# gizatechxyz/LuminAIR

Hardware: AMD Instinct MI355X
Metric: proofs/sec, 2^20-row Add trace (higher is better)
Workload: dtype u32 (M31/QM31 field arithmetic)

## Files before the change

### luminair_amd/csrc/fft_fixed.h

```cpp
#pragma once
#include "kernels.h"

namespace lmn {

bool launch_fft_fixed_pass(bool inverse, uint32_t* data, uint64_t col_stride, const uint32_t* src, uint64_t src_stride, int lo,
                           int rbits, int cb, int log_n, const TwPtrs& tw, uint32_t scale_log, int ncols, int cpb,
                           uint32_t h_off, int xcd_swizzle, bool zero_extended_top, lmn_stream_t s);
bool launch_interp_extend_fixed(uint32_t* coeffs, uint64_t coeff_stride, uint32_t* lde, uint64_t lde_stride, int log_n,
                                const TwPtrs& itw, const TwPtrs& tw_ext, int ncols, lmn_stream_t s);
bool launch_fft_rows_fixed(uint32_t* coeffs, uint64_t col_stride, const uint32_t* rows, uint64_t n_rows, int ncols, int log_n,
                           const PadRow& pad, uint32_t* bad_flag, uint32_t bad_value, const TwPtrs& itw, lmn_stream_t s);

}
```

### luminair_amd/csrc/fft_fixed.hip

```cpp
#include "fft_fixed.h"

#include <algorithm>

#include "issue_phases.h"
#include "launch_util.h"

namespace lmn {

LMN_HD constexpr uint32_t fx_pad(uint32_t e) { return e + (e >> 5); }

#if !defined(LMN_EMU) && !defined(LMN_BATCH)
#define LMN_BOUNDS(n) __launch_bounds__(n)
#else
#define LMN_BOUNDS(n)
#endif

struct GTile {
#if defined(__HIP_DEVICE_COMPILE__) && !defined(LMN_EMU)
  __amdgpu_buffer_rsrc_t r;
#else
  uint32_t* p;
#endif
};
LMN_D GTile gtile(const uint32_t* p) {
// ... 254 lines not shown
}

struct TwD {
  const uint32_t* l[MAX_LOG];
};
static TwD doubled(const TwPtrs& tw) {
  TwD t{};
  for (int i = 0; i < MAX_LOG; ++i) t.l[i] = tw.d[i];
  return t;
}

template <bool INV, int RBITS, int CB, bool LO0, bool ZX = false>
LMN_KERNEL LMN_BOUNDS((FxShape<RBITS, CB, LO0>::NT))
k_fft_fx(uint32_t* data, uint64_t col_stride, const uint32_t* src, uint64_t src_stride, int lo_arg, TwD tw, uint32_t scale_log,
         int ncols, int cpb, uint32_t h_off, int xcd_swizzle) {
  using S = FxShape<RBITS, CB, LO0>;
  LMN_DYN_SMEM(uint32_t, sm);
  const int lo = LO0 ? 0 : lo_arg;
  uint32_t tile = blockIdx.x;
  if (xcd_swizzle && (gridDim.x & 7u) == 0u) tile = (blockIdx.x & 7u) * (gridDim.x >> 3) + (blockIdx.x >> 3);
  const uint32_t q = tile & ((1u << (lo - CB)) - 1u);
  const uint32_t Hl = tile >> (lo - CB);
  const uint64_t base = ((uint64_t)Hl << (lo + RBITS)) + ((uint64_t)q << CB);
  const uint32_t H = Hl + h_off;
  for (int cc = 0; cc < cpb; ++cc) {
    const int c = (int)blockIdx.y * cpb + cc;
    if (c >= ncols) break;
    uint32_t* col = data + (uint64_t)c * col_stride + base;
    const uint32_t* scol = src + (uint64_t)c * src_stride + base;
    fx_steps<S, INV, 0, true, true, false, ZX>(sm, sm, col, scol, lo, H, tw.l, scale_log, nullptr, threadIdx.x);
  }
}

template <int RBITS>
LMN_KERNEL LMN_BOUNDS((FxShape<RBITS, 4, false>::NT))
k_fft_interp_extend_fx(uint32_t* coeffs, uint64_t coeff_stride, uint32_t* lde, uint64_t lde_stride, TwD itw, TwD tw,
                       uint32_t scale_log) {
  using S = FxShape<RBITS, 4, false>;
  constexpr int LO = 12;
  LMN_DYN_SMEM(uint32_t, sm);
  uint32_t* A = sm;
  uint32_t* B = sm + S::LDS_WORDS;
  uint32_t tile = blockIdx.x;
  if ((gridDim.x & 7u) == 0u) tile = (blockIdx.x & 7u) * (gridDim.x >> 3) + (blockIdx.x >> 3);
  const uint64_t base = (uint64_t)tile << 4;
  const uint64_t n_words = 1ull << (LO + RBITS);
  uint32_t* ccol = coeffs + (uint64_t)blockIdx.y * coeff_stride + base;
  uint32_t* lcol = lde + (uint64_t)blockIdx.y * lde_stride + base;
  fx_steps<S, true, 0, true, true, true>(B, B, ccol, ccol, LO, 0u, itw.l, scale_log, A, threadIdx.x);
  for (uint32_t h = 0; h < 2; ++h)
    fx_steps<S, false, 0, false, true, false>(A, B, lcol + h * n_words, nullptr, LO, h, tw.l, 0u, nullptr, threadIdx.x);
}

template <int COLS>
LMN_KERNEL LMN_BOUNDS((COLS / 2) * 256)
k_fft_rows_fx(uint32_t* coeffs, uint64_t col_stride, const uint32_t* __restrict__ rows, uint64_t n_rows, int ncols, PadRow pad,
              uint32_t* __restrict__ bad_flag, uint32_t bad_value, TwD itw, uint32_t n_groups) {
  using S = FxShape<12, 0, true>;
  constexpr uint32_t NT = (uint32_t)S::NT, TILE = 1u << 12, GROUPS = COLS / 2;
  static_assert(NT == 256, "one lane group per tile");
  LMN_DYN_SMEM(uint32_t, sm);
  uint32_t tile = blockIdx.x / n_groups, ygrp = blockIdx.x % n_groups;
  if ((gridDim.x & 7u) == 0u && ((gridDim.x / n_groups) & 7u) == 0u) {
    const uint32_t x = blockIdx.x & 7u, sq = blockIdx.x >> 3;
    tile = (sq / n_groups) * 8u + x;
    ygrp = sq % n_groups;
  }
  const int c0 = (int)ygrp * COLS;
  const int ncb = ncols - c0 < COLS ? ncols - c0 : COLS;
  const uint64_t row0 = (uint64_t)tile << 12;
  {
    constexpr int BATCH = 8;
    constexpr uint32_t CELLS = TILE * COLS, STEP = GROUPS * NT;
    for (uint32_t k0 = threadIdx.x; k0 < CELLS; k0 += BATCH * STEP) {
      uint32_t v[BATCH];
#pragma unroll
      for (int j = 0; j < BATCH; ++j) {
        const uint32_t k = k0 + (uint32_t)j * STEP;
        const uint32_t r = k / COLS, c = k % COLS;
        const uint64_t gr = row0 + r;
        v[j] = 0u;
        if ((int)c < ncb) v[j] = gr < n_rows ? rows[gr * (uint64_t)ncols + (uint32_t)c0 + c] : pad.v[(uint32_t)c0 + c];
      }
#pragma unroll
// ... 82 lines not shown
    switch (rbits) {
      case 5: LMN_FX_CASE(5, 5, false);
      case 6: LMN_FX_CASE(6, 5, false);
      case 7: LMN_FX_CASE(7, 5, false);
      default: return false;
    }
  }
  if (cb == 4 && lo >= 4) {
    switch (rbits) {
      case 6: LMN_FX_CASE(6, 4, false);
      case 7: LMN_FX_CASE(7, 4, false);
      case 8: LMN_FX_CASE(8, 4, false);
      case 9: LMN_FX_CASE(9, 4, false);
      case 10: LMN_FX_CASE(10, 4, false);
      default: return false;
    }
  }
  return false;
#undef LMN_FX_CASE
}

bool launch_fft_fixed_pass(bool inverse, uint32_t* data, uint64_t col_stride, const uint32_t* src, uint64_t src_stride, int lo,
                           int rbits, int cb, int log_n, const TwPtrs& tw, uint32_t scale_log, int ncols, int cpb,
                           uint32_t h_off, int xcd_swizzle, bool zero_extended_top, lmn_stream_t s) {
  static const bool off = env_set("LMN_NO_FFT_FIXED");
  if (off || !tw.d[0]) return false;
  if (zero_extended_top && (inverse || lo + rbits != log_n)) return false;
  return inverse ? dispatch_fx<true>(data, col_stride, src, src_stride, lo, rbits, cb, log_n, tw, scale_log, ncols, cpb, h_off,
                                     xcd_swizzle, false, s)
                 : dispatch_fx<false>(data, col_stride, src, src_stride, lo, rbits, cb, log_n, tw, scale_log, ncols, cpb, h_off,
                                      xcd_swizzle, zero_extended_top, s);
}

template <int RBITS>
static void launch_ie(uint32_t* coeffs, uint64_t coeff_stride, uint32_t* lde, uint64_t lde_stride, const TwPtrs& itw,
                      const TwPtrs& tw_ext, uint32_t scale_log, int ncols, lmn_stream_t s) {
  using S = FxShape<RBITS, 4, false>;
  const size_t smem = (size_t)8 * S::LDS_WORDS;
#if !defined(LMN_EMU) && !defined(LMN_BATCH)
  if (smem > 64 * 1024) allow_big_lds((const void*)k_fft_interp_extend_fx<RBITS>, 160 * 1024);
#endif
  LMN_LAUNCH((k_fft_interp_extend_fx<RBITS>), dim3(1u << (12 - 4), (unsigned)ncols), dim3(S::NT), smem, s, coeffs, coeff_stride,
             lde, lde_stride, doubled(itw), doubled(tw_ext), scale_log);
}

bool launch_interp_extend_fixed(uint32_t* coeffs, uint64_t coeff_stride, uint32_t* lde, uint64_t lde_stride, int log_n,
                                const TwPtrs& itw, const TwPtrs& tw_ext, int ncols, lmn_stream_t s) {
  static const bool off = env_set("LMN_NO_FFT_FIXED");
  if (off || !itw.d[0] || !tw_ext.d[0]) return false;
  const uint32_t scale_log = (uint32_t)((31 - (log_n % 31)) % 31);
  switch (log_n - 12) {
    case 6: launch_ie<6>(coeffs, coeff_stride, lde, lde_stride, itw, tw_ext, scale_log, ncols, s); return true;
    case 7: launch_ie<7>(coeffs, coeff_stride, lde, lde_stride, itw, tw_ext, scale_log, ncols, s); return true;
    case 8: launch_ie<8>(coeffs, coeff_stride, lde, lde_stride, itw, tw_ext, scale_log, ncols, s); return true;
    case 9: launch_ie<9>(coeffs, coeff_stride, lde, lde_stride, itw, tw_ext, scale_log, ncols, s); return true;
    default: return false;
  }
}

}
```

### luminair_amd/csrc/kernels.h

```cpp
#pragma once
#include "blake2s.h"
#include "field.h"

namespace lmn {

constexpr int MAX_LOG = 30;

struct TwPtrs {
  const uint32_t* l[MAX_LOG];
  const uint32_t* d[MAX_LOG];
};

struct PadRow {
  uint32_t v[32];
};
void launch_transpose_pad(const uint32_t* rows, uint64_t n_rows, int ncols, int log_size, uint32_t* cols,
                          const PadRow& pad, uint32_t* bad_flag , lmn_stream_t s);
void launch_transpose_pad_rows(const uint32_t* rows, uint64_t n_rows, int ncols, int log_size, uint32_t* cols,
                               uint64_t out_stride, uint64_t blk_row0, uint64_t blk_rows, const PadRow& pad, uint32_t* bad_flag,
                               lmn_stream_t s,
                               uint32_t bad_value = 1u );
constexpr int CHUNK_ROWS = 256;
constexpr int CHUNK_MAX_COLS = 30;
void launch_rows_chunk(const uint32_t* chunk, uint64_t r0, uint64_t n, int ncols, uint32_t* cols, uint64_t stride,
                       const PadRow& pad, uint32_t* bad_word, lmn_stream_t s);
constexpr int PREPARE_MAX_LUT_COLS = 6;
struct PrepareCols {
  const uint32_t* lut[PREPARE_MAX_LUT_COLS];
  uint32_t n[PREPARE_MAX_LUT_COLS];
  int n_luts;
  uint32_t* range_check;
  uint32_t range_n;
};
void launch_settings_prepare(const PrepareCols& cols, uint32_t* flag, lmn_stream_t s);

int launch_ifft(uint32_t* dst, uint64_t dst_stride, const uint32_t* src, uint64_t src_stride, int ncols, int log_n,
                const TwPtrs& itw, lmn_stream_t s);
int launch_fft(uint32_t* dst, uint64_t dst_stride, const uint32_t* src, uint64_t src_stride, int log_src, int ncols,
               int log_n, const TwPtrs& tw, lmn_stream_t s);
bool fft_interp_extend_supported(int log_n);
int launch_interp_extend(uint32_t* coeffs, uint64_t coeff_stride, const uint32_t* evals, uint64_t evals_stride, uint32_t* lde,
                         uint64_t lde_stride, int ncols, int log_n, const TwPtrs& itw, const TwPtrs& tw_ext, lmn_stream_t s);
struct PadRow;
bool launch_interp_extend_rows(uint32_t* coeffs, uint64_t coeff_stride, const uint32_t* rows, uint64_t n_rows, const PadRow& pad,
                               uint32_t* bad_flag, uint32_t bad_value, uint32_t* lde, uint64_t lde_stride, int ncols, int log_n,
                               const TwPtrs& itw, const TwPtrs& tw_ext, lmn_stream_t s);
int launch_fft_block(uint32_t* dst, uint64_t dst_stride, const uint32_t* src, uint64_t src_stride, int log_src, int ncols,
                     int log_n, int log_blocks, uint32_t block, const TwPtrs& tw, lmn_stream_t s);
struct PackSel {
  uint32_t blk[8][2];
};
void launch_pack_blocks(const uint32_t* src, uint64_t src_stride, uint32_t* dst, uint32_t block_rows, int ncols, int nsel,
                        int world, const PackSel& sel, lmn_stream_t s);
void launch_unpack_blocks(const uint32_t* packed, uint32_t* cols, uint64_t col_stride, uint32_t block_rows, int ncols, int world,
                          lmn_stream_t s);
void launch_fft_simple(uint32_t* data, uint64_t col_stride, int ncols, int log_n, const TwPtrs& tw, bool inverse,
                       lmn_stream_t s);
void launch_extend(const uint32_t* src, uint64_t src_stride, int log_src, uint32_t* dst, uint64_t dst_stride,
                   int log_dst, int ncols, lmn_stream_t s);

void launch_bit_reverse(uint32_t* data, uint64_t col_stride, int ncols, int log_n, lmn_stream_t s);
int decompose_num_blocks(int log_n);
void launch_decompose(const uint32_t* f, int log_n, uint32_t* g, QM31* lambda_out, QM31* scratch, lmn_stream_t s);
void launch_batch_inverse_m31(const uint32_t* src, uint32_t* dst, uint64_t col_stride, int ncols, int log_n,
                              unsigned long long* n_zero, lmn_stream_t s);
void launch_batch_inverse_qm31(const uint32_t* src, uint32_t* dst, int log_n, unsigned long long* n_zero, lmn_stream_t s);

void launch_merkle_layer(const uint32_t* prev, const uint32_t* const* cols, int ncols, uint32_t size, uint32_t* out,
                         lmn_stream_t s);

struct DevChannel {
  uint32_t digest[8];
  uint32_t n_sent;
  uint32_t variant;
};
// ... 263 lines not shown
  uint32_t n;
};
int logup_num_blocks(uint32_t n);
void launch_logup_fracs(const LogupArgs& a, lmn_stream_t s);
void launch_logup_reduce(const uint32_t* partials, int nblocks, uint32_t n_inv, QM31* claimed_out, lmn_stream_t s);
void launch_logup_scan(const QM31* last_tmp, QM31* claimed_shift, int log_size, uint32_t* out_cols ,
                       QM31* blocksums, lmn_stream_t s, bool derive_claim = false, uint32_t n_inv = 0);
int logup_scan_num_blocks(int log_size);

struct CompositionArgs {
  int kind;
  int log_size;
  int eval_log;
  uint32_t row0, n_rows;
  uint64_t stride;
  const uint32_t* main;
  const uint32_t* inter;
  const uint32_t* prev_last;
  uint32_t* out;
  int accumulate;
  QM31 z, alpha;
  QM31 z2, alpha2;
  const DevElems* d_elems;
  int es2;
  const uint32_t* pre;
  const uint32_t* pre2;
  const QM31* claimed_shift;
  QM31 coeff[16];
  const QM31* d_coeff;
  uint32_t zinv[2];
};
void launch_composition(const CompositionArgs& a, lmn_stream_t s);
void launch_secure_add(uint32_t* out, const uint32_t* in, uint64_t n_words, lmn_stream_t s);

struct EvalJob {
  const uint32_t* coeffs;
  int log_n;
  int point;
  int owner = -1;
};
constexpr int EVAL_LB = 10;
void launch_eval_at_point(const EvalJob* jobs, int njobs, const QM31* lo_tab, const QM31* hi_tab, uint32_t hi_stride,
                          int max_log, QM31* partial_out , int max_chunks, lmn_stream_t s,
                          uint32_t shard_rank = 0, uint32_t shard_world = 1);
int eval_num_chunks(int log_n);
void launch_eval_tables(const QM31* maps, int maps_stride, int npoints, QM31* lo_tab, QM31* hi_tab, uint32_t hi_n,
                        int hi_bits, lmn_stream_t s);
void launch_eval_reduce(const EvalJob* jobs, int njobs, const QM31* partial, int max_chunks, QM31* out,
                        lmn_stream_t s);

constexpr int QUOT_MAX_BATCH = 4;
constexpr int QUOT_MAX_ENTRIES = 512;
struct QuotEntry {
  const uint32_t* col;
  QM31 c;
};
struct QuotDev {
  QM31 A[QUOT_MAX_BATCH], B[QUOT_MAX_BATCH], batch_coeff[QUOT_MAX_BATCH];
  CM31 prx[QUOT_MAX_BATCH], pry[QUOT_MAX_BATCH], pix[QUOT_MAX_BATCH], piy[QUOT_MAX_BATCH];
};
struct QuotientArgs {
  int log_size;
  uint32_t row0;
  int log_rows;
  uint64_t out_stride;
  int nbatch;
// ... 44 lines not shown
```

### luminair_amd/csrc/kernels_fft.hip

```cpp
#include "kernels_common.h"

namespace lmn {

constexpr int FFT_MAX_STAGES = 4;
struct FftStagePlan {
  int lo, hi, cb;
  int nst;
  int first[FFT_MAX_STAGES];
  int R[FFT_MAX_STAGES];
  int xcd_swizzle;
};

LMN_HD uint32_t fft_lds_pad(uint32_t e) { return e + (e >> 5); }

template <int N>
LMN_D void m_mul_phased(const uint32_t (&x)[N], const uint32_t (&w)[N], uint32_t (&out)[N]) {
  uint64_t pr[N];
  uint32_t hi[N], s[N], s2[N];
  LMN_PHASE_PORT0();
#pragma unroll
  for (int k = 0; k < N; ++k) pr[k] = (uint64_t)x[k] * (uint64_t)w[k];
#pragma unroll
  for (int k = 0; k < N; ++k) hi[k] = (uint32_t)(pr[k] >> 31);
  LMN_PHASE_ANY();
// ... 179 lines not shown
    case 2: fft_stage<2, INV>(sm_in, sm_out, col, scol, src_len, base, lo, hi, cb, first_layer, H, from_global, to_global, tw, scale, keep); break;
    case 3: fft_stage<3, INV>(sm_in, sm_out, col, scol, src_len, base, lo, hi, cb, first_layer, H, from_global, to_global, tw, scale, keep); break;
    default: fft_stage<4, INV>(sm_in, sm_out, col, scol, src_len, base, lo, hi, cb, first_layer, H, from_global, to_global, tw, scale, keep); break;
  }
}

template <bool INV>
LMN_KERNEL k_fft_staged(uint32_t* data, uint64_t col_stride, const uint32_t* src, uint64_t src_stride,
                        uint64_t src_len, FftStagePlan pl, TwPtrs tw, uint32_t scale, int ncols, int cpb,
                        uint32_t h_off) {
  LMN_DYN_SMEM(uint32_t, sm);
  uint32_t tile = blockIdx.x;
  if (pl.xcd_swizzle && (gridDim.x & 7u) == 0u) tile = (blockIdx.x & 7u) * (gridDim.x >> 3) + (blockIdx.x >> 3);
  const uint32_t q = tile & ((1u << (pl.lo - pl.cb)) - 1u);
  const uint32_t Hl = tile >> (pl.lo - pl.cb);
  const uint64_t base = ((uint64_t)Hl << pl.hi) + ((uint64_t)q << pl.cb);
  const uint32_t H = Hl + h_off;
  for (int cc = 0; cc < cpb; ++cc) {
    const int c = blockIdx.y * cpb + cc;
    if (c >= ncols) break;
    uint32_t* col = data + (uint64_t)c * col_stride;
    const uint32_t* scol = src + (uint64_t)c * src_stride;
    for (int k = 0; k < pl.nst; ++k) {
      const int s = INV ? k : pl.nst - 1 - k;
      const bool fg = k == 0, tg = k == pl.nst - 1;
      fft_stage_dispatch<INV>(pl.R[s], sm, sm, col, scol, src_len, base, pl.lo, pl.hi, pl.cb, pl.first[s], H, fg, tg, tw, scale);
      __syncthreads();
    }
  }
}

LMN_KERNEL k_fft_interp_extend(uint32_t* coeffs, uint64_t coeff_stride, const uint32_t* src, uint64_t src_stride,
                               uint32_t* lde, uint64_t lde_stride, FftStagePlan pl, TwPtrs itw, TwPtrs tw, uint32_t scale,
                               int ncols, int cpb) {
  LMN_DYN_SMEM(uint32_t, sm);
  const uint32_t tile_elems = 1u << (pl.hi - pl.lo + pl.cb);
  uint32_t* A = sm;
  uint32_t* B = sm + fft_lds_pad(tile_elems) + 1u;
  uint32_t tile = blockIdx.x;
  if (pl.xcd_swizzle && (gridDim.x & 7u) == 0u) tile = (blockIdx.x & 7u) * (gridDim.x >> 3) + (blockIdx.x >> 3);
  const uint64_t base = (uint64_t)tile << pl.cb;
  const uint64_t n_words = 1ull << pl.hi;
  for (int cc = 0; cc < cpb; ++cc) {
    const int c = blockIdx.y * cpb + cc;
    if (c >= ncols) break;
    uint32_t* ccol = coeffs + (uint64_t)c * coeff_stride;
    const uint32_t* scol = src + (uint64_t)c * src_stride;
    uint32_t* lcol = lde + (uint64_t)c * lde_stride;
    for (int k = 0; k < pl.nst; ++k) {
      const bool fg = k == 0, tg = k == pl.nst - 1;
      fft_stage_dispatch<true>(pl.R[k], B, B, ccol, scol, n_words, base, pl.lo, pl.hi, pl.cb, pl.first[k], 0u, fg, tg, itw, scale,
                               tg ? A : nullptr);
      __syncthreads();
    }
    for (uint32_t h = 0; h < 2; ++h) {
      for (int k = 0; k < pl.nst; ++k) {
        const int s = pl.nst - 1 - k;
        const bool tg = k == pl.nst - 1;
        fft_stage_dispatch<false>(pl.R[s], k == 0 ? A : B, B, lcol + h * n_words, lcol, 0, base, pl.lo, pl.hi, pl.cb, pl.first[s], h,
                                  false, tg, tw, 1u);
        __syncthreads();
      }
    }
  }
}

struct FftPass {
  int lo, hi, cb;
};
constexpr int FFT_LOW_BITS = 12;
constexpr int FFT_HIGH_BITS = 10;
constexpr int FFT_HIGH_CB = 4;

static int plan_passes(int log_n, FftPass* out) {
  int n = 0;
  int lo = 0;
  int hi = log_n < FFT_LOW_BITS ? log_n : FFT_LOW_BITS;
  out[n++] = {0, hi, 0};
  lo = hi;
  while (lo < log_n) {
    int rem = log_n - lo;
    int npass = (rem + FFT_HIGH_BITS - 1) / FFT_HIGH_BITS;
    int take = (rem + npass - 1) / npass;
    out[n++] = {lo, lo + take, (take == 5 || (npass > 1 && take <= 7)) ? 5 : FFT_HIGH_CB};
    lo += take;
  }
  return n;
}
// ... 38 lines not shown
    const uint32_t scale_log = scale == 1u ? 0u : (uint32_t)__builtin_ctz(scale);
    if (launch_fft_fixed_pass(INV, data, col_stride, psrc, pstride, p.lo, rbits, p.cb, log_n, tw, scale_log, ncols, cpb,
                              block_index << (log_n - p.hi), pl.xcd_swizzle, !full, s))
      return;
  }
  unsigned gy = (unsigned)((ncols + cpb - 1) / cpb);
  const int threads = (int)std::min<uint32_t>(TPB, std::max<uint32_t>(64u, tile_elems >> 4));
  LMN_LAUNCH(k_fft_staged<INV>, dim3(tiles, gy), dim3(threads), smem, s, data, col_stride, psrc, pstride, plen, pl, tw,
             scale, ncols, cpb, block_index << (log_n - p.hi));
}

template <bool INV>
static int run_fft(uint32_t* data, uint64_t col_stride, const uint32_t* src, uint64_t src_stride, int log_src,
                    int ncols, int log_n, const TwPtrs& tw, lmn_stream_t s, uint32_t block_index = 0) {
  if (log_n < 1) throw LmnError(-100, "fft: log_n < 1");
  FftPass passes[8];
  int np = plan_passes(log_n, passes);
  for (int k = 0; k < np; ++k) {
    const FftPass& p = INV ? passes[k] : passes[np - 1 - k];
    bool last = INV && k == np - 1;
    uint32_t scale = last ? inv_pow2(log_n) : 1u;
    const uint32_t* psrc = k == 0 ? src : data;
    uint64_t pstride = k == 0 ? src_stride : col_stride;
    uint64_t plen = k == 0 ? (1ull << log_src) : (1ull << log_n);
    launch_staged_pass<INV>(data, col_stride, psrc, pstride, plen, p, log_n, tw, scale, ncols, s, block_index);
  }
  return np;
}

bool fft_interp_extend_supported(int log_n) {
  static const bool off = env_set("LMN_NO_FFT_FUSION");
  return !off && log_n > FFT_LOW_BITS && log_n - FFT_LOW_BITS <= FFT_HIGH_BITS - 1;
}
static void interp_extend_tail(uint32_t* coeffs, uint64_t coeff_stride, uint32_t* lde, uint64_t lde_stride, int ncols, int log_n,
                               const TwPtrs& itw, const TwPtrs& tw_ext, lmn_stream_t s) {
  const FftPass low{0, FFT_LOW_BITS, 0};
  FftStagePlan pl{};
  pl.lo = FFT_LOW_BITS;
  pl.hi = log_n;
  pl.cb = FFT_HIGH_CB;
  split_stages(pl);
  pl.xcd_swizzle = 1;
  const uint32_t tile_elems = 1u << (log_n - FFT_LOW_BITS + FFT_HIGH_CB);
  const size_t smem = (size_t)8 * (tile_elems + (tile_elems >> 5) + 1);
  const unsigned tiles = 1u << (FFT_LOW_BITS - FFT_HIGH_CB);
  int cpb = 1;
  const int threads = (int)std::min<uint32_t>(TPB, std::max<uint32_t>(64u, tile_elems >> 4));
#if !defined(LMN_EMU) && !defined(LMN_BATCH)
  if (smem > 64 * 1024) allow_big_lds((const void*)k_fft_interp_extend, 160 * 1024);
#endif
  if (!launch_interp_extend_fixed(coeffs, coeff_stride, lde, lde_stride, log_n, itw, tw_ext, ncols, s))
    LMN_LAUNCH(k_fft_interp_extend, dim3(tiles, (unsigned)((ncols + cpb - 1) / cpb)), dim3(threads), smem, s, coeffs,
               coeff_stride, coeffs, coeff_stride, lde, lde_stride, pl, itw, tw_ext, inv_pow2(log_n), ncols, cpb);
  launch_staged_pass<false>(lde, lde_stride, lde, lde_stride, 2ull << log_n, low, log_n + 1, tw_ext, 1u, ncols, s);
}

int launch_interp_extend(uint32_t* coeffs, uint64_t coeff_stride, const uint32_t* evals, uint64_t evals_stride, uint32_t* lde,
                         uint64_t lde_stride, int ncols, int log_n, const TwPtrs& itw, const TwPtrs& tw_ext, lmn_stream_t s) {
  if (!fft_interp_extend_supported(log_n)) throw LmnError(-100, "interp_extend: unsupported size");
  const FftPass low{0, FFT_LOW_BITS, 0};
  launch_staged_pass<true>(coeffs, coeff_stride, evals, evals_stride, 1ull << log_n, low, log_n, itw, 1u, ncols, s);
  interp_extend_tail(coeffs, coeff_stride, lde, lde_stride, ncols, log_n, itw, tw_ext, s);
  return 3;
}

bool launch_interp_extend_rows(uint32_t* coeffs, uint64_t coeff_stride, const uint32_t* rows, uint64_t n_rows, const PadRow& pad,
                               uint32_t* bad_flag, uint32_t bad_value, uint32_t* lde, uint64_t lde_stride, int ncols, int log_n,
                               const TwPtrs& itw, const TwPtrs& tw_ext, lmn_stream_t s) {
  static_assert(FFT_LOW_BITS == 12, "k_fft_rows_fx is the 12-layer contiguous pass");
  if (!fft_interp_extend_supported(log_n)) return false;
  if (!launch_fft_rows_fixed(coeffs, coeff_stride, rows, n_rows, ncols, log_n, pad, bad_flag, bad_value, itw, s)) return false;
  interp_extend_tail(coeffs, coeff_stride, lde, lde_stride, ncols, log_n, itw, tw_ext, s);
  return true;
}

int launch_ifft(uint32_t* dst, uint64_t dst_stride, const uint32_t* src, uint64_t src_stride, int ncols, int log_n,
                const TwPtrs& itw, lmn_stream_t s) {
  return run_fft<true>(dst, dst_stride, src, src_stride, log_n, ncols, log_n, itw, s);
}
int launch_fft(uint32_t* dst, uint64_t dst_stride, const uint32_t* src, uint64_t src_stride, int log_src, int ncols,
               int log_n, const TwPtrs& tw, lmn_stream_t s) {
  return run_fft<false>(dst, dst_stride, src, src_stride, log_src, ncols, log_n, tw, s);
}

template <int G>
LMN_KERNEL k_fft_top_block(uint32_t* __restrict__ dst, uint64_t dst_stride, const uint32_t* __restrict__ src,
                           uint64_t src_stride, uint64_t src_len, int log_n, uint32_t block, TwPtrs tw) {
  const uint64_t S = 1ull << (log_n - G);
  const uint64_t t = (uint64_t)blockIdx.x * blockDim.x + threadIdx.x;
  if (t >= S) return;
  const uint32_t* scol = src + (uint64_t)blockIdx.y * src_stride;
  uint32_t v[1 << G];
#pragma unroll
  for (int c = 0; c < (1 << G); ++c) {
    const uint64_t idx = (uint64_t)c * S + t;
    v[c] = idx < src_len ? scol[idx] : 0u;
// ... 140 lines not shown
```

### luminair_amd/csrc/kernels_quotient.hip

```cpp
#include "kernels_common.h"
#include "constraints.h"

namespace lmn {

LMN_D uint32_t prev_row_storage(uint32_t s, int eval_log, int log_size) {
  const int hb = eval_log - 1;
  const uint32_t low = s & 1u;
  uint32_t t = s >> 1;
  if (hb == 0) return s;
  const uint32_t mask = (1u << hb) - 1u;
  const uint32_t d = 1u << (eval_log - log_size - 1);
  uint32_t j = __brev(t) >> (32 - hb);
  j = (low ? j + d : j - d) & mask;
  t = __brev(j) >> (32 - hb);
  return (t << 1) | low;
}

struct ConsAcc {
  QAcc acc;
  const QM31* coeff;
  int k;
  LMN_HD void bump() {
    ++k;
    if (k % 3 == 0) qacc_fold(acc);
// ... 74 lines not shown
  QM31 r = q_mul_m(qacc_reduce(ca.acc), a.zinv[(s >> a.log_size) & 1u]);
  if (a.accumulate) {
    r.a = m_add(r.a, ld_ub(a.out, s));
    r.b = m_add(r.b, ld_ub(a.out + E, s));
    r.c = m_add(r.c, ld_ub(a.out + 2 * E, s));
    r.d = m_add(r.d, ld_ub(a.out + 3 * E, s));
  }
  st_ub(a.out, s, r.a);
  st_ub(a.out + E, s, r.b);
  st_ub(a.out + 2 * E, s, r.c);
  st_ub(a.out + 3 * E, s, r.d);
}

void launch_composition(const CompositionArgs& a, lmn_stream_t s) {
  if (a.eval_log != a.log_size + 1) throw LmnError(-100, "composition: eval domain must be log_size+1");
  if (a.n_rows == 0 || (uint64_t)a.row0 + a.n_rows > (1ull << a.eval_log) || a.stride < a.n_rows || !a.prev_last)
    throw LmnError(-100, "composition: bad row block");
  dim3 g(cdiv(a.n_rows, TPB)), b(TPB);
#define LMN_COMP_CASE(K) case K: LMN_LAUNCH(k_composition<K>, g, b, 0, s, a); break;
  switch (composition_shape(a.kind)) {
    LMN_COMP_CASE(0) LMN_COMP_CASE(1) LMN_COMP_CASE(2) LMN_COMP_CASE(3) LMN_COMP_CASE(4) LMN_COMP_CASE(5) LMN_COMP_CASE(6)
    LMN_COMP_CASE(7) LMN_COMP_CASE(8) LMN_COMP_CASE(13) LMN_COMP_CASE(14) LMN_COMP_CASE(15) LMN_COMP_CASE(16)
    default: throw LmnError(-100, "composition: unsupported component kind");
  }
#undef LMN_COMP_CASE
}

LMN_KERNEL k_secure_add(uint32_t* __restrict__ out, const uint32_t* __restrict__ in, uint64_t n) {
  uint64_t i = (uint64_t)blockIdx.x * blockDim.x + threadIdx.x;
  if (i < n) out[i] = m_add(out[i], in[i]);
}
void launch_secure_add(uint32_t* out, const uint32_t* in, uint64_t n_words, lmn_stream_t s) {
  LMN_LAUNCH(k_secure_add, dim3(cdiv(n_words, TPB)), dim3(TPB), 0, s, out, in, n_words);
}

constexpr int EVAL_HI_PER_CHUNK = 8;
LMN_HD int eval_num_chunks_hd(int log_n) {
  if (log_n <= EVAL_LB) return 1;
  int total_hi = 1 << (log_n - EVAL_LB);
  int hpc = total_hi < EVAL_HI_PER_CHUNK ? total_hi : EVAL_HI_PER_CHUNK;
  return total_hi / hpc;
}
int eval_num_chunks(int log_n) { return eval_num_chunks_hd(log_n); }

LMN_KERNEL k_eval_at_point(const EvalJob* __restrict__ jobs, const QM31* __restrict__ lo_tab,
                           const QM31* __restrict__ hi_tab, uint32_t hi_stride, QM31* __restrict__ partial_out,
                           int max_chunks, uint32_t shard_rank, uint32_t shard_world) {
  LMN_SHARED QM31 red[TPB];
  const EvalJob job = jobs[blockIdx.y];
  const int chunk = blockIdx.x;
  const int nchunks = eval_num_chunks_hd(job.log_n);
  if (chunk >= nchunks) return;
  if (shard_world > 1) {
    const uint32_t owner = job.owner >= 0 ? (uint32_t)job.owner
                           : (uint32_t)nchunks >= shard_world ? (uint32_t)chunk / ((uint32_t)nchunks / shard_world) : (uint32_t)chunk;
    if (owner != shard_rank) {
      if (threadIdx.x == 0) partial_out[(uint64_t)blockIdx.y * max_chunks + chunk] = q_zero();
      return;
    }
  }
  const int lb = job.log_n < EVAL_LB ? job.log_n : EVAL_LB;
  const uint32_t lo_n = 1u << lb;
  const uint32_t total_hi = 1u << (job.log_n - lb);
  const uint32_t hpc = total_hi / (uint32_t)nchunks;
  const QM31* L = lo_tab + ((uint64_t)job.point << EVAL_LB);
  const QM31* Hh = hi_tab + (uint64_t)job.point * hi_stride;
// ... 271 lines not shown
```

### luminair_amd/csrc/phase_composition.cpp

```cpp
#include "prove_run.h"

namespace lmn {

void Context::run_composition(ProofRun& r) {
  LMN_RUN_ALIASES(r);
  int n_total = 0;
  for (auto& ci : inst) n_total += constraint_layout(*ci.spec, cfg.protocol_variant).n_protocol;
  std::vector<QM31> powers(std::max(n_total, 1));
  if (!r.dev_fs) {
    comp_alpha = channel.draw_felt();
    powers[0] = q_one();
    for (int k = 1; k < n_total; ++k) powers[k] = q_mul(powers[k - 1], comp_alpha);
  }
  size_t inst_index = 0;
  {
    StageTimer st(this, log, stream_, C_COMPOSITION);
    std::map<int, uint32_t*> sub;
    const int sg = shard_.active ? shard_.g : 0;
    int k0 = 0;
    for (auto& ci : inst) {
      int e = ci.log_size + 1;
      uint64_t E = 1ull << e;
      bool first = sub.find(e) == sub.end();
      if (first) sub[e] = arena_.alloc_words(4 * E);
      CompositionArgs a{};
      a.kind = ci.spec->kind;
      a.log_size = ci.log_size;
      a.eval_log = e;
      a.main = tree1.cols[ci.main_start].lde;
      a.inter = tree2.cols[ci.inter_start].lde;
      const uint32_t* pre_e[2] = {ci.pre_idx[0] >= 0 ? tree0.cols[ci.pre_idx[0]].lde : nullptr,
                                  ci.pre_idx[1] >= 0 ? tree0.cols[ci.pre_idx[1]].lde : nullptr};
      if (lb != 1) {
        auto on_eval_domain = [&](const uint32_t* coeffs, int ncols) {
          const uint64_t rows = E >> sg;
          uint32_t* ev = arena_.alloc_words((size_t)ncols * rows);
          StageTimer t(this, log, stream_, C_FFT);
          if (sg == 0)
            timings.fft_launches += launch_fft(ev, E, coeffs, 1ull << ci.log_size, ci.log_size, ncols, e, tw(e), stream_);
          else
            timings.fft_launches += launch_fft_block(ev, rows, coeffs, 1ull << ci.log_size, ci.log_size, ncols, e, sg,
                                                     shard_.rank, tw(e), stream_);
          timings.fft_bytes += (uint64_t)ncols * (4ull << ci.log_size) + (uint64_t)ncols * 4ull * rows;
          timings.fft_butterflies += (uint64_t)ncols * (rows / 2) * (uint64_t)e;
          return (const uint32_t*)ev;
        };
        a.main = on_eval_domain(tree1.cols[ci.main_start].coeffs, ci.spec->n_cols);
        a.inter = on_eval_domain(tree2.cols[ci.inter_start].coeffs, 4 * ci.spec->n_rel);
        for (int k = 0; k < 2; ++k)
          if (ci.pre_idx[k] >= 0) pre_e[k] = on_eval_domain(tree0.cols[ci.pre_idx[k]].coeffs, 1);
      }
// ... 22 lines not shown
      a.out = sub[e];
      a.accumulate = first ? 0 : 1;
      a.z = elems.z[ELEMS_NODE];
      a.alpha = elems.alpha[ELEMS_NODE];
      for (int j = 0; j < ci.spec->n_rel; ++j)
        if (ci.spec->rel_elems[j] != ELEMS_NODE) {
          a.z2 = elems.z[ci.spec->rel_elems[j]];
          a.alpha2 = elems.alpha[ci.spec->rel_elems[j]];
        }
      a.pre = pre_e[0];
      a.pre2 = pre_e[1];
      a.claimed_shift = ci.d_claimed_shift;
      const ConstraintLayout L = constraint_layout(*ci.spec, cfg.protocol_variant);
      if (r.dev_fs) {
        a.d_coeff = r.d_coeff + 16 * inst_index;
        a.d_elems = &r.d_report->elems;
        a.es2 = ELEMS_NODE;
        for (int j = 0; j < ci.spec->n_rel; ++j)
          if (ci.spec->rel_elems[j] != ELEMS_NODE) a.es2 = ci.spec->rel_elems[j];
      } else {
        for (int k = 0; k < L.n_kernel; ++k) {
          a.coeff[k] = L.proto_index[k] < 0 ? q_zero() : powers[n_total - 1 - (k0 + L.proto_index[k])];
          if (L.neg[k]) a.coeff[k] = q_neg(a.coeff[k]);
        }
      }
      ++inst_index;
      k0 += L.n_protocol;
      for (int b = 0; b < 2; ++b) {
        Pt p = domain_point(e, (uint32_t)b << ci.log_size);
        uint32_t x = p.x;
        for (int k = 0; k < ci.log_size - 1; ++k) x = m_sub(m_dbl(m_sqr(x)), 1u);
        a.zinv[b] = m_inv(x);
      }
      launch_composition(a, stream_);
    }
    if (shard_.active)
      for (auto& kv : sub) gather_columns(kv.second, 1ull << kv.first, 4, (1ull << kv.first) >> sg);
    uint32_t* cur = nullptr;
    CommitOut comp_out;
    int cur_log = 0;
    for (auto& kv : sub) {
      int e = kv.first;
      uint64_t E = 1ull << e;
      uint32_t* vals = kv.second;
      if (cur) {
        uint32_t* ext = arena_.alloc_words(4 * E);
        StageTimer t(this, log, stream_, C_FFT);
        timings.fft_launches += launch_fft(ext, E, cur, 1ull << cur_log, cur_log, 4, e, tw(e), stream_);
        timings.fft_bytes += 4ull * (4ull << cur_log) + 4ull * 4ull * E;
        timings.fft_butterflies += 4ull * (E / 2) * (uint64_t)e;
        launch_secure_add(vals, ext, 4 * E, stream_);
      }
      if (e == comp_log) {
        comp_out = interpolate_for_commit(vals, vals, 4, e);
      } else {
        StageTimer t(this, log, stream_, C_FFT);
        timings.fft_launches += launch_ifft(vals, E, vals, E, 4, e, itw(e), stream_);
        timings.fft_bytes += 4ull * 8ull * E;
        timings.fft_butterflies += 4ull * (E / 2) * (uint64_t)e;
      }
      cur = vals;
      cur_log = e;
    }
    if (cur_log != comp_log) throw LmnError(LMN_ERR_INTERNAL, "composition size mismatch");
    for (int k = 0; k < 4; ++k)
      tree3.cols.push_back({comp_log, cur + ((uint64_t)k << comp_log), comp_out.lde ? comp_out.lde + (uint64_t)k * comp_out.stride : nullptr,
                            comp_out.sharded, comp_out.owner_of(k)});
  }
  {
    StageTimer st(this, log, stream_, C_COMP_COMMIT);
    if (r.dev_fs) {
      ChanStep step;
      plan_oods_step(r, step);
      lde_and_merkle(tree3, false, r.d_chan, &step);
      hm.mark("composition enqueued (device transcript)");
      return;
    }
// ... 11 lines not shown
```

Baseline: 770.6.

## Evaluate composition on half domain and fix top coefficient via probe dot

Composition polynomial evaluation is restricted to half the rows plus one probe row, and the full-degree interpolation is reconstructed from a half-size IFFT. The single top coefficient is recovered with a probe dot-product correction kernel, and the LDE is extended fourfold directly from the half-size coefficients. This cuts composition evaluation and FFT work roughly in half but adds probe-dot, add-cols and fix-up kernels, and it relies on subtle algebraic correctness.

Result: faster. 794.7, median of 6 (+3.1%).

```diff
diff --git a/luminair_amd/csrc/fft_fixed.h b/luminair_amd/csrc/fft_fixed.h
--- a/luminair_amd/csrc/fft_fixed.h
+++ b/luminair_amd/csrc/fft_fixed.h
@@ -7,7 +7,7 @@
                            int rbits, int cb, int log_n, const TwPtrs& tw, uint32_t scale_log, int ncols, int cpb,
                            uint32_t h_off, int xcd_swizzle, bool zero_extended_top, lmn_stream_t s);
 bool launch_interp_extend_fixed(uint32_t* coeffs, uint64_t coeff_stride, uint32_t* lde, uint64_t lde_stride, int log_n,
-                                const TwPtrs& itw, const TwPtrs& tw_ext, int ncols, lmn_stream_t s);
+                                const TwPtrs& itw, const TwPtrs& tw_ext, int ncols, int n_ext, lmn_stream_t s);
 bool launch_fft_rows_fixed(uint32_t* coeffs, uint64_t col_stride, const uint32_t* rows, uint64_t n_rows, int ncols, int log_n,
                            const PadRow& pad, uint32_t* bad_flag, uint32_t bad_value, const TwPtrs& itw, lmn_stream_t s);
 
diff --git a/luminair_amd/csrc/fft_fixed.hip b/luminair_amd/csrc/fft_fixed.hip
--- a/luminair_amd/csrc/fft_fixed.hip
+++ b/luminair_amd/csrc/fft_fixed.hip
@@ -310,13 +310,11 @@
   }
 }
 
-template <int RBITS>
-LMN_KERNEL LMN_BOUNDS((FxShape<RBITS, 4, false>::NT))
-k_fft_interp_extend_fx(uint32_t* coeffs, uint64_t coeff_stride, uint32_t* lde, uint64_t lde_stride, TwD itw, TwD tw,
-                       uint32_t scale_log) {
+template <int RBITS, int NH>
+LMN_D void fx_interp_extend_tile(uint32_t* sm, uint32_t* coeffs, uint64_t coeff_stride, uint32_t* lde, uint64_t lde_stride,
+                                 const TwD& itw, const TwD& tw, uint32_t scale_log) {
   using S = FxShape<RBITS, 4, false>;
   constexpr int LO = 12;
-  LMN_DYN_SMEM(uint32_t, sm);
   uint32_t* A = sm;
   uint32_t* B = sm + S::LDS_WORDS;
   uint32_t tile = blockIdx.x;
@@ -326,8 +324,25 @@
   uint32_t* ccol = coeffs + (uint64_t)blockIdx.y * coeff_stride + base;
   uint32_t* lcol = lde + (uint64_t)blockIdx.y * lde_stride + base;
   fx_steps<S, true, 0, true, true, true>(B, B, ccol, ccol, LO, 0u, itw.l, scale_log, A, threadIdx.x);
-  for (uint32_t h = 0; h < 2; ++h)
+#pragma unroll
+  for (uint32_t h = 0; h < (uint32_t)NH; ++h)
     fx_steps<S, false, 0, false, true, false>(A, B, lcol + h * n_words, nullptr, LO, h, tw.l, 0u, nullptr, threadIdx.x);
+}
+
+template <int RBITS>
+LMN_KERNEL LMN_BOUNDS((FxShape<RBITS, 4, false>::NT))
+k_fft_interp_extend_fx(uint32_t* coeffs, uint64_t coeff_stride, uint32_t* lde, uint64_t lde_stride, TwD itw, TwD tw,
+                       uint32_t scale_log) {
+  LMN_DYN_SMEM(uint32_t, sm);
+  fx_interp_extend_tile<RBITS, 2>(sm, coeffs, coeff_stride, lde, lde_stride, itw, tw, scale_log);
+}
+
+template <int RBITS>
+LMN_KERNEL LMN_BOUNDS((FxShape<RBITS, 4, false>::NT))
+k_fft_interp_quarters_fx(uint32_t* coeffs, uint64_t coeff_stride, uint32_t* lde, uint64_t lde_stride, TwD itw, TwD tw,
+                         uint32_t scale_log) {
+  LMN_DYN_SMEM(uint32_t, sm);
+  fx_interp_extend_tile<RBITS, 4>(sm, coeffs, coeff_stride, lde, lde_stride, itw, tw, scale_log);
 }
 
 template <int COLS>
@@ -476,30 +491,44 @@
                                       xcd_swizzle, zero_extended_top, s);
 }
 
-template <int RBITS>
+template <int RBITS, int NH>
 static void launch_ie(uint32_t* coeffs, uint64_t coeff_stride, uint32_t* lde, uint64_t lde_stride, const TwPtrs& itw,
                       const TwPtrs& tw_ext, uint32_t scale_log, int ncols, lmn_stream_t s) {
   using S = FxShape<RBITS, 4, false>;
   const size_t smem = (size_t)8 * S::LDS_WORDS;
+  if constexpr (NH == 2) {
 #if !defined(LMN_EMU) && !defined(LMN_BATCH)
-  if (smem > 64 * 1024) allow_big_lds((const void*)k_fft_interp_extend_fx<RBITS>, 160 * 1024);
-#endif
-  LMN_LAUNCH((k_fft_interp_extend_fx<RBITS>), dim3(1u << (12 - 4), (unsigned)ncols), dim3(S::NT), smem, s, coeffs, coeff_stride,
-             lde, lde_stride, doubled(itw), doubled(tw_ext), scale_log);
+    if (smem > 64 * 1024) allow_big_lds((const void*)k_fft_interp_extend_fx<RBITS>, 160 * 1024);
+#endif
+    LMN_LAUNCH((k_fft_interp_extend_fx<RBITS>), dim3(1u << (12 - 4), (unsigned)ncols), dim3(S::NT), smem, s, coeffs,
+               coeff_stride, lde, lde_stride, doubled(itw), doubled(tw_ext), scale_log);
+  } else {
+#if !defined(LMN_EMU) && !defined(LMN_BATCH)
+    if (smem > 64 * 1024) allow_big_lds((const void*)k_fft_interp_quarters_fx<RBITS>, 160 * 1024);
+#endif
+    LMN_LAUNCH((k_fft_interp_quarters_fx<RBITS>), dim3(1u << (12 - 4), (unsigned)ncols), dim3(S::NT), smem, s, coeffs,
+               coeff_stride, lde, lde_stride, doubled(itw), doubled(tw_ext), scale_log);
+  }
 }
 
 bool launch_interp_extend_fixed(uint32_t* coeffs, uint64_t coeff_stride, uint32_t* lde, uint64_t lde_stride, int log_n,
-                                const TwPtrs& itw, const TwPtrs& tw_ext, int ncols, lmn_stream_t s) {
+                                const TwPtrs& itw, const TwPtrs& tw_ext, int ncols, int n_ext, lmn_stream_t s) {
   static const bool off = env_set("LMN_NO_FFT_FIXED");
-  if (off || !itw.d[0] || !tw_ext.d[0]) return false;
+  if (off || !itw.d[0] || !tw_ext.d[0] || (n_ext != 2 && n_ext != 4)) return false;
   const uint32_t scale_log = (uint32_t)((31 - (log_n % 31)) % 31);
+#define LMN_IE_CASE(RB)                                                                                        \
+  case RB:                                                                                                     \
+    if (n_ext == 2) launch_ie<RB, 2>(coeffs, coeff_stride, lde, lde_stride, itw, tw_ext, scale_log, ncols, s); \
+    else launch_ie<RB, 4>(coeffs, coeff_stride, lde, lde_stride, itw, tw_ext, scale_log, ncols, s);            \
+    return true
   switch (log_n - 12) {
-    case 6: launch_ie<6>(coeffs, coeff_stride, lde, lde_stride, itw, tw_ext, scale_log, ncols, s); return true;
-    case 7: launch_ie<7>(coeffs, coeff_stride, lde, lde_stride, itw, tw_ext, scale_log, ncols, s); return true;
-    case 8: launch_ie<8>(coeffs, coeff_stride, lde, lde_stride, itw, tw_ext, scale_log, ncols, s); return true;
-    case 9: launch_ie<9>(coeffs, coeff_stride, lde, lde_stride, itw, tw_ext, scale_log, ncols, s); return true;
+    LMN_IE_CASE(6);
+    LMN_IE_CASE(7);
+    LMN_IE_CASE(8);
+    LMN_IE_CASE(9);
     default: return false;
   }
-}
-
-}
+#undef LMN_IE_CASE
+}
+
+}
diff --git a/luminair_amd/csrc/kernels.h b/luminair_amd/csrc/kernels.h
--- a/luminair_amd/csrc/kernels.h
+++ b/luminair_amd/csrc/kernels.h
@@ -41,6 +41,11 @@
 bool fft_interp_extend_supported(int log_n);
 int launch_interp_extend(uint32_t* coeffs, uint64_t coeff_stride, const uint32_t* evals, uint64_t evals_stride, uint32_t* lde,
                          uint64_t lde_stride, int ncols, int log_n, const TwPtrs& itw, const TwPtrs& tw_ext, lmn_stream_t s);
+int launch_interp_extend_half(uint32_t* coeffs, uint64_t coeff_stride, const uint32_t* evals, uint64_t evals_stride,
+                              uint32_t* lde, uint64_t lde_stride, int ncols, int log_half, const TwPtrs& itw_full,
+                              const TwPtrs& tw_ext, lmn_stream_t s);
+int launch_interp_extend_half_finish(uint32_t* lde, uint64_t lde_stride, int ncols, int log_half, const TwPtrs& tw_ext,
+                                     lmn_stream_t s);
 struct PadRow;
 bool launch_interp_extend_rows(uint32_t* coeffs, uint64_t coeff_stride, const uint32_t* rows, uint64_t n_rows, const PadRow& pad,
                                uint32_t* bad_flag, uint32_t bad_value, uint32_t* lde, uint64_t lde_stride, int ncols, int log_n,
@@ -370,6 +375,31 @@
 };
 void launch_composition(const CompositionArgs& a, lmn_stream_t s);
 void launch_secure_add(uint32_t* out, const uint32_t* in, uint64_t n_words, lmn_stream_t s);
+void launch_add_cols(uint32_t* out, uint64_t out_stride, const uint32_t* in, uint64_t in_stride, uint64_t n, int ncols,
+                     lmn_stream_t s);
+
+struct ProbeMaps {
+  uint32_t m[MAX_LOG];
+};
+constexpr int PROBE_CHUNK_LOG = 12;
+inline uint32_t probe_dot_blocks(int log_n) { return log_n > PROBE_CHUNK_LOG ? 1u << (log_n - PROBE_CHUNK_LOG) : 1u; }
+void launch_probe_dot(const uint32_t* coeffs, uint64_t stride, int log_n, const ProbeMaps& pm, uint32_t* partial,
+                      uint32_t* tail_out, lmn_stream_t s);
+struct CompHalfFix {
+  uint32_t* coeffs;
+  uint64_t coeff_stride;
+  uint32_t* lde;
+  uint64_t lde_stride;
+  int log_half;
+  const uint32_t* part_g;
+  uint32_t n_g;
+  const uint32_t* part_f;
+  uint32_t n_f;
+  const uint32_t* probe;
+  const uint32_t* w_top;
+  const uint32_t* w_ext;
+};
+void launch_comp_half_fix(const CompHalfFix& f, lmn_stream_t s);
 
 struct EvalJob {
   const uint32_t* coeffs;
diff --git a/luminair_amd/csrc/kernels_fft.hip b/luminair_amd/csrc/kernels_fft.hip
--- a/luminair_amd/csrc/kernels_fft.hip
+++ b/luminair_amd/csrc/kernels_fft.hip
@@ -235,7 +235,7 @@
 
 LMN_KERNEL k_fft_interp_extend(uint32_t* coeffs, uint64_t coeff_stride, const uint32_t* src, uint64_t src_stride,
                                uint32_t* lde, uint64_t lde_stride, FftStagePlan pl, TwPtrs itw, TwPtrs tw, uint32_t scale,
-                               int ncols, int cpb) {
+                               int ncols, int cpb, uint32_t n_ext) {
   LMN_DYN_SMEM(uint32_t, sm);
   const uint32_t tile_elems = 1u << (pl.hi - pl.lo + pl.cb);
   uint32_t* A = sm;
@@ -256,7 +256,7 @@
                                tg ? A : nullptr);
       __syncthreads();
     }
-    for (uint32_t h = 0; h < 2; ++h) {
+    for (uint32_t h = 0; h < n_ext; ++h) {
       for (int k = 0; k < pl.nst; ++k) {
         const int s = pl.nst - 1 - k;
         const bool tg = k == pl.nst - 1;
@@ -361,9 +361,8 @@
   static const bool off = env_set("LMN_NO_FFT_FUSION");
   return !off && log_n > FFT_LOW_BITS && log_n - FFT_LOW_BITS <= FFT_HIGH_BITS - 1;
 }
-static void interp_extend_tail(uint32_t* coeffs, uint64_t coeff_stride, uint32_t* lde, uint64_t lde_stride, int ncols, int log_n,
-                               const TwPtrs& itw, const TwPtrs& tw_ext, lmn_stream_t s) {
-  const FftPass low{0, FFT_LOW_BITS, 0};
+static void interp_extend_strided(uint32_t* coeffs, uint64_t coeff_stride, uint32_t* lde, uint64_t lde_stride, int ncols,
+                                  int log_n, const TwPtrs& itw, const TwPtrs& tw_ext, uint32_t n_ext, lmn_stream_t s) {
   FftStagePlan pl{};
   pl.lo = FFT_LOW_BITS;
   pl.hi = log_n;
@@ -378,9 +377,14 @@
 #if !defined(LMN_EMU) && !defined(LMN_BATCH)
   if (smem > 64 * 1024) allow_big_lds((const void*)k_fft_interp_extend, 160 * 1024);
 #endif
-  if (!launch_interp_extend_fixed(coeffs, coeff_stride, lde, lde_stride, log_n, itw, tw_ext, ncols, s))
+  if (!launch_interp_extend_fixed(coeffs, coeff_stride, lde, lde_stride, log_n, itw, tw_ext, ncols, (int)n_ext, s))
     LMN_LAUNCH(k_fft_interp_extend, dim3(tiles, (unsigned)((ncols + cpb - 1) / cpb)), dim3(threads), smem, s, coeffs,
-               coeff_stride, coeffs, coeff_stride, lde, lde_stride, pl, itw, tw_ext, inv_pow2(log_n), ncols, cpb);
+               coeff_stride, coeffs, coeff_stride, lde, lde_stride, pl, itw, tw_ext, inv_pow2(log_n), ncols, cpb, n_ext);
+}
+static void interp_extend_tail(uint32_t* coeffs, uint64_t coeff_stride, uint32_t* lde, uint64_t lde_stride, int ncols, int log_n,
+                               const TwPtrs& itw, const TwPtrs& tw_ext, lmn_stream_t s) {
+  const FftPass low{0, FFT_LOW_BITS, 0};
+  interp_extend_strided(coeffs, coeff_stride, lde, lde_stride, ncols, log_n, itw, tw_ext, 2u, s);
   launch_staged_pass<false>(lde, lde_stride, lde, lde_stride, 2ull << log_n, low, log_n + 1, tw_ext, 1u, ncols, s);
 }
 
@@ -391,6 +395,22 @@
   launch_staged_pass<true>(coeffs, coeff_stride, evals, evals_stride, 1ull << log_n, low, log_n, itw, 1u, ncols, s);
   interp_extend_tail(coeffs, coeff_stride, lde, lde_stride, ncols, log_n, itw, tw_ext, s);
   return 3;
+}
+
+int launch_interp_extend_half(uint32_t* coeffs, uint64_t coeff_stride, const uint32_t* evals, uint64_t evals_stride,
+                              uint32_t* lde, uint64_t lde_stride, int ncols, int log_half, const TwPtrs& itw_full,
+                              const TwPtrs& tw_ext, lmn_stream_t s) {
+  if (!fft_interp_extend_supported(log_half)) throw LmnError(-100, "interp_extend_half: unsupported size");
+  const FftPass low{0, FFT_LOW_BITS, 0};
+  launch_staged_pass<true>(coeffs, coeff_stride, evals, evals_stride, 1ull << log_half, low, log_half, itw_full, 1u, ncols, s);
+  interp_extend_strided(coeffs, coeff_stride, lde, lde_stride, ncols, log_half, itw_full, tw_ext, 4u, s);
+  return 2;
+}
+int launch_interp_extend_half_finish(uint32_t* lde, uint64_t lde_stride, int ncols, int log_half, const TwPtrs& tw_ext,
+                                     lmn_stream_t s) {
+  const FftPass low{0, FFT_LOW_BITS, 0};
+  launch_staged_pass<false>(lde, lde_stride, lde, lde_stride, 4ull << log_half, low, log_half + 2, tw_ext, 1u, ncols, s);
+  return 1;
 }
 
 bool launch_interp_extend_rows(uint32_t* coeffs, uint64_t coeff_stride, const uint32_t* rows, uint64_t n_rows, const PadRow& pad,
diff --git a/luminair_amd/csrc/kernels_quotient.hip b/luminair_amd/csrc/kernels_quotient.hip
--- a/luminair_amd/csrc/kernels_quotient.hip
+++ b/luminair_amd/csrc/kernels_quotient.hip
@@ -130,6 +130,95 @@
 }
 void launch_secure_add(uint32_t* out, const uint32_t* in, uint64_t n_words, lmn_stream_t s) {
   LMN_LAUNCH(k_secure_add, dim3(cdiv(n_words, TPB)), dim3(TPB), 0, s, out, in, n_words);
+}
+
+LMN_KERNEL k_add_cols(uint32_t* __restrict__ out, uint64_t out_stride, const uint32_t* __restrict__ in, uint64_t in_stride,
+                      uint64_t n) {
+  const uint64_t i = (uint64_t)blockIdx.x * blockDim.x + threadIdx.x;
+  if (i >= n) return;
+  uint32_t* o = out + (uint64_t)blockIdx.y * out_stride + i;
+  *o = m_add(*o, in[(uint64_t)blockIdx.y * in_stride + i]);
+}
+void launch_add_cols(uint32_t* out, uint64_t out_stride, const uint32_t* in, uint64_t in_stride, uint64_t n, int ncols,
+                     lmn_stream_t s) {
+  LMN_LAUNCH(k_add_cols, dim3(cdiv(n, TPB), (unsigned)ncols), dim3(TPB), 0, s, out, out_stride, in, in_stride, n);
+}
+
+LMN_D uint32_t probe_basis(const ProbeMaps& pm, uint32_t v, int k0, int nbits) {
+  uint32_t acc = 1u;
+  for (int k = 0; k < nbits; ++k)
+    if ((v >> k) & 1u) acc = m_mul(acc, pm.m[k0 + k]);
+  return acc;
+}
+LMN_D uint32_t probe_block_sum(uint32_t* red, uint32_t v) {
+  red[threadIdx.x] = v;
+  __syncthreads();
+  for (int st = TPB / 2; st > 0; st >>= 1) {
+    if ((int)threadIdx.x < st) red[threadIdx.x] = m_add(red[threadIdx.x], red[threadIdx.x + st]);
+    __syncthreads();
+  }
+  const uint32_t r = red[0];
+  __syncthreads();
+  return r;
+}
+LMN_KERNEL k_probe_dot(const uint32_t* __restrict__ coeffs, uint64_t stride, int log_n, ProbeMaps pm,
+                       uint32_t* __restrict__ partial, uint32_t* __restrict__ tail_out) {
+  LMN_SHARED uint32_t red[TPB];
+  const uint32_t* __restrict__ col = coeffs + (uint64_t)blockIdx.y * stride;
+  const uint64_t n = 1ull << log_n;
+  const uint64_t j0 = (uint64_t)blockIdx.x << PROBE_CHUNK_LOG;
+  const int lane_bits = log_n < 8 ? log_n : 8;
+  const int mid_bits = log_n < PROBE_CHUNK_LOG ? (log_n > 8 ? log_n - 8 : 0) : PROBE_CHUNK_LOG - 8;
+  uint32_t acc = 0u;
+  for (uint32_t i = 0; i < (1u << mid_bits); ++i) {
+    const uint64_t j = j0 + ((uint64_t)i << 8) + threadIdx.x;
+    if (threadIdx.x < (1u << lane_bits) && j < n) acc = m_add(acc, m_mul(col[j], probe_basis(pm, i, 8, mid_bits)));
+  }
+  acc = m_mul(acc, probe_basis(pm, threadIdx.x, 0, lane_bits));
+  if (log_n > PROBE_CHUNK_LOG) acc = m_mul(acc, probe_basis(pm, blockIdx.x, PROBE_CHUNK_LOG, log_n - PROBE_CHUNK_LOG));
+  const uint32_t sum = probe_block_sum(red, acc);
+  if (threadIdx.x == 0) {
+    partial[(uint64_t)blockIdx.y * gridDim.x + blockIdx.x] = sum;
+    if (tail_out && blockIdx.x == 0) tail_out[blockIdx.y] = col[n];
+  }
+}
+void launch_probe_dot(const uint32_t* coeffs, uint64_t stride, int log_n, const ProbeMaps& pm, uint32_t* partial,
+                      uint32_t* tail_out, lmn_stream_t s) {
+  if (log_n < 0 || log_n >= MAX_LOG) throw LmnError(-100, "probe_dot: bad size");
+  LMN_LAUNCH(k_probe_dot, dim3(probe_dot_blocks(log_n), 4), dim3(TPB), 0, s, coeffs, stride, log_n, pm, partial, tail_out);
+}
+
+LMN_KERNEL k_comp_half_fix(CompHalfFix f) {
+  LMN_SHARED uint32_t red[TPB];
+  const uint32_t c4 = blockIdx.y;
+  uint32_t acc = 0u;
+  for (uint32_t k = threadIdx.x; k < f.n_g; k += blockDim.x) acc = m_add(acc, f.part_g[(uint64_t)c4 * f.n_g + k]);
+  for (uint32_t k = threadIdx.x; k < f.n_f; k += blockDim.x) acc = m_sub(acc, f.part_f[(uint64_t)c4 * f.n_f + k]);
+  const uint32_t diff = m_sub(probe_block_sum(red, acc), f.probe[c4]);
+  const uint32_t w = f.w_top[0];
+  const uint32_t c = m_mul(diff, m_inv(m_add(w, w)));
+  const uint64_t N = 1ull << f.log_half;
+  uint32_t* __restrict__ col = f.coeffs + (uint64_t)c4 * f.coeff_stride;
+  const uint64_t gid = (uint64_t)blockIdx.x * blockDim.x + threadIdx.x, gstep = (uint64_t)gridDim.x * blockDim.x;
+  if (gid == 0) col[0] = m_sub(col[0], m_mul(w, c));
+  for (uint64_t i = gid; i < N; i += gstep) col[N + i] = i == 0 ? c : 0u;
+  if (f.lde) {
+    uint32_t* __restrict__ l = f.lde + (uint64_t)c4 * f.lde_stride;
+    const uint64_t per = N >> 12;
+    for (uint64_t i = gid; i < 4 * per; i += gstep) {
+      const uint32_t h = (uint32_t)(i / per);
+      const uint32_t we = f.w_ext[h >> 1];
+      const uint32_t kappa = m_sub((h & 1u) ? m_neg(we) : we, w);
+      uint32_t* p = l + (uint64_t)h * N + ((i % per) << 12);
+      *p = m_add(*p, m_mul(c, kappa));
+    }
+  }
+}
+void launch_comp_half_fix(const CompHalfFix& f, lmn_stream_t s) {
+  if (f.log_half < 0 || (f.lde && f.log_half < 12)) throw LmnError(-100, "comp_half_fix: bad size");
+  const uint64_t N = 1ull << f.log_half;
+  const unsigned gx = (unsigned)std::min<uint64_t>(std::max<uint64_t>(N / (4 * TPB), 1), 256);
+  LMN_LAUNCH(k_comp_half_fix, dim3(gx, 4), dim3(TPB), 0, s, f);
 }
 
 constexpr int EVAL_HI_PER_CHUNK = 8;
diff --git a/luminair_amd/csrc/phase_composition.cpp b/luminair_amd/csrc/phase_composition.cpp
--- a/luminair_amd/csrc/phase_composition.cpp
+++ b/luminair_amd/csrc/phase_composition.cpp
@@ -17,6 +17,12 @@
     StageTimer st(this, log, stream_, C_COMPOSITION);
     std::map<int, uint32_t*> sub;
     const int sg = shard_.active ? shard_.g : 0;
+#ifdef LMN_BATCH
+    const bool half = false;
+#else
+    const bool half = !shard_.active && lb == 1 && fft_interp_extend_supported(comp_log - 1) &&
+                      env_int("LMN_COMP_FULL_DOMAIN", 0) == 0;
+#endif
     int k0 = 0;
     for (auto& ci : inst) {
       int e = ci.log_size + 1;
@@ -105,6 +111,7 @@
         for (int k = 0; k < ci.log_size - 1; ++k) x = m_sub(m_dbl(m_sqr(x)), 1u);
         a.zinv[b] = m_inv(x);
       }
+      if (half) a.n_rows = (uint32_t)(E / 2) + 1;
       launch_composition(a, stream_);
     }
     if (shard_.active)
@@ -116,6 +123,65 @@
       int e = kv.first;
       uint64_t E = 1ull << e;
       uint32_t* vals = kv.second;
+      if (half) {
+        const int lh = e - 1;
+        const uint64_t N = E / 2;
+        const Pt pp = domain_point(e, (uint32_t)N);
+        ProbeMaps pm{};
+        pm.m[0] = pp.y;
+        pm.m[1] = pp.x;
+        for (int k = 2; k < e; ++k) pm.m[k] = m_sub(m_dbl(m_sqr(pm.m[k - 1])), 1u);
+        CompHalfFix f{};
+        if (cur) {
+          uint32_t* ext = arena_.alloc_words(4 * N);
+          uint32_t* part = arena_.alloc_words(4 * (size_t)probe_dot_blocks(cur_log));
+          StageTimer t(this, log, stream_, C_FFT);
+          timings.fft_launches += launch_fft_block(ext, N, cur, 1ull << cur_log, cur_log, 4, e, 1, 0, tw(e), stream_);
+          timings.fft_bytes += 4ull * (4ull << cur_log) + 4ull * 4ull * N;
+          timings.fft_butterflies += 4ull * (N / 2) * (uint64_t)lh;
+          launch_add_cols(vals, E, ext, N, N, 4, stream_);
+          launch_probe_dot(cur, 1ull << cur_log, cur_log, pm, part, nullptr, stream_);
+          f.part_f = part;
+          f.n_f = probe_dot_blocks(cur_log);
+        }
+        uint32_t* lde = nullptr;
+        {
+          StageTimer t(this, log, stream_, C_FFT);
+          timings.fft_bytes += 4ull * 8ull * N;
+          timings.fft_butterflies += 4ull * (N / 2) * (uint64_t)lh;
+          if (e == comp_log) {
+            lde = arena_.alloc_words(4 * 4 * N);
+            timings.fft_launches += launch_interp_extend_half(vals, E, vals, E, lde, 4 * N, 4, lh, itw(e), tw(e + 1), stream_);
+            timings.fft_bytes += 4ull * 20ull * N;
+            timings.fft_butterflies += 4ull * 2ull * N * (uint64_t)lh;
+          } else {
+            if (lh >= 1) timings.fft_launches += launch_ifft(vals, E, vals, E, 4, lh, itw(e), stream_);
+          }
+        }
+        uint32_t* part_g = arena_.alloc_words(4 * (size_t)probe_dot_blocks(lh) + 4);
+        uint32_t* probe = part_g + 4 * (size_t)probe_dot_blocks(lh);
+        launch_probe_dot(vals, E, lh, pm, part_g, probe, stream_);
+        f.coeffs = vals;
+        f.coeff_stride = E;
+        f.lde = lde;
+        f.lde_stride = 4 * N;
+        f.log_half = lh;
+        f.part_g = part_g;
+        f.n_g = probe_dot_blocks(lh);
+        f.probe = probe;
+        f.w_top = tw(e).l[e - 1];
+        f.w_ext = tw(e + 1).l[e - 1];
+        launch_comp_half_fix(f, stream_);
+        if (lde) {
+          StageTimer t(this, log, stream_, C_FFT);
+          timings.fft_launches += launch_interp_extend_half_finish(lde, 4 * N, 4, lh, tw(e + 1), stream_);
+          comp_out.lde = lde;
+          comp_out.stride = 4 * N;
+        }
+        cur = vals;
+        cur_log = e;
+        continue;
+      }
       if (cur) {
         uint32_t* ext = arena_.alloc_words(4 * E);
         StageTimer t(this, log, stream_, C_FFT);
```
